# amin-abouee/apex-solver

Measured on AMD Instinct MI355X. Metric: ms per LM iter (Jacobian+Schur+solve), lower is better.
Workload: dtype f64; 1 GPU; final-13682 synthetic (13682 cameras / 4456117 landmarks / 28966251 observations); optimization_type=selfcal, camera_dof=9, schur_variant=sparse, s_tile_rows=856, s_tiles=8071, s_tiles_touched=4284, etree_levels=41, border_cameras=0, schur_form=4, variant_asked=Sparse, reason=, variant_choice=direct, parallelism=landmark-shard x1

## Files before the change

### apex-solver_amd/csrc/chol_kernels.hip

```cpp
#include <hip/hip_runtime.h>
#include <stdint.h>

#include "chol_kernels.h"
#include "device_reduce.hpp"
#include "tile_kernel_defs.h"
#include <algorithm>

namespace apex {

constexpr int BS = 16;
constexpr int NBK = NB / BS;
constexpr int BP = 18;
constexpr int BSZ = BS * BP;
constexpr int NLB = NBK * (NBK + 1) / 2;

__device__ __forceinline__ int bidx(int bi, int bj) { return bi * (bi + 1) / 2 + bj; }

__device__ __forceinline__ double readlane_f64(double v, int src) {
    const int lo = __builtin_amdgcn_readlane(__double2loint(v), src);
    const int hi = __builtin_amdgcn_readlane(__double2hiint(v), src);
    return __hiloint2double(hi, lo);
}

__device__ __forceinline__ double4_t blk_mma_nt(const double* X, const double* Y, double4_t acc, int lr, int lk, double sgn) {
// ... 176 lines not shown
                if (j + 2 < BS) {
                    const double dd = readlane_f64(Dm[(j + 2) >> 2], 16 * ((j + 2) & 3) + j + 2);
                    const double a0 = readlane_f64(l0, 16 * q0 + j + 2), a1 = readlane_f64(l1, 16 * q1 + j + 2);
                    dnext = fma(-a1, a1, fma(-a0, a0, dd));
                    Dm = __builtin_amdgcn_mfma_f64_16x16x4f64(-la, la, Dm, 0, 0, 0);
                    Xm = __builtin_amdgcn_mfma_f64_16x16x4f64(-la, xb, Xm, 0, 0, 0);
                }
            }
            double* D = sA + bidx(kb, kb) * BSZ;
            double* Xd = sD + kb * BSZ;
#pragma unroll
            for (int r = 0; r < 4; ++r) {
                const int c = lk + 4 * r;
                D[lr * BP + c] = lr >= c ? Ls[r] : 0.0;
                Xd[c * BP + lr] = Xs[r];
            }
            if (isbad) *bad = 1;
            POTRF_STAMP();
        } else if (helper) {
            if (kb >= 1) {
                const int ks = kb - 1;
                for (int i = kb + 1 + hid; i < NBK; i += NH) {
                    double* Cb = sA + bidx(i, kb) * BSZ;
                    double4_t acc = blk_load_cd(Cb, lr, lk);
                    acc = blk_mma_nt(sA + bidx(i, ks) * BSZ, sA + bidx(kb, ks) * BSZ, acc, lr, lk, -1.0);
                    blk_store_cd(Cb, acc, lr, lk, 1.0);
                }
                const int m = NBK - 1 - kb;
                const int n_upd = m * (m + 1) / 2;
                for (int t = hid; t < n_upd; t += NH) {
                    int ii = 0;
                    while ((ii + 1) * (ii + 2) / 2 <= t) ++ii;
                    const int jj = t - ii * (ii + 1) / 2;
                    const int i = kb + 1 + ii, j = kb + 1 + jj;
                    double* Cb = sA + bidx(i, j) * BSZ;
                    double4_t acc = blk_load_cd(Cb, lr, lk);
                    acc = blk_mma_nt(sA + bidx(i, ks) * BSZ, sA + bidx(j, ks) * BSZ, acc, lr, lk, -1.0);
                    blk_store_cd(Cb, acc, lr, lk, 1.0);
                }
                const int r = ks;
                int nt = 0;
                for (int j = hid; j < r; j += NH, ++nt) {
                    double4_t acc = (double4_t){0.0, 0.0, 0.0, 0.0};
                    for (int k = j; k < r; ++k) {
                        const double* Y = (k == j) ? (sD + j * BSZ) : (sA + bidx(k, j) * BSZ);
                        acc = blk_mma_nn(sA + bidx(r, k) * BSZ, Y, acc, lr, lk);
                    }
                    T[nt] = acc;
                }
            }
        }
        __syncthreads();
        POTRF_STAMP();
        if (helper && kb >= 1) {
            const int r = kb - 1;
            int nt = 0;
            for (int j = hid; j < r; j += NH, ++nt) blk_store_cd(sA + bidx(r, j) * BSZ, T[nt], lr, lk, -1.0);
        }
        {
            const int m = NBK - 1 - kb;
            if (w == 0) {
                if (m > 0) {
                    double* N = sA + bidx(kb + 1, kb) * BSZ;
                    double4_t Lt = (double4_t){0.0, 0.0, 0.0, 0.0};
                    Lt = blk_mma_nt(sD + kb * BSZ, N, Lt, lr, lk, 1.0);
                    Dm = blk_load_cd_sym(sA + bidx(kb + 1, kb + 1) * BSZ, lr, lk);
#pragma unroll
                    for (int r = 0; r < 4; ++r) N[lr * BP + lk + 4 * r] = Lt[r];
#pragma unroll
                    for (int r = 0; r < 4; ++r) Dm = __builtin_amdgcn_mfma_f64_16x16x4f64(-Lt[r], Lt[r], Dm, 0, 0, 0);
                }
            } else if (helper) {
                const int t0 = m > 0 ? 1 : 0;
                for (int t = t0 + hid; t < m + kb; t += NH) {
                    if (t < m) {
                        double* P = sA + bidx(kb + 1 + t, kb) * BSZ;
                        double4_t acc = (double4_t){0.0, 0.0, 0.0, 0.0};
                        acc = blk_mma_nt(P, sD + kb * BSZ, acc, lr, lk, 1.0);
                        blk_store_cd(P, acc, lr, lk, 1.0);
                    } else {
                        const int k = t - m;
                        double* Bk = sA + bidx(kb, k) * BSZ;
                        blk_to_tile<COH>(Bk, A, rA, kb, k, lane, 64);
                        double4_t acc = (double4_t){0.0, 0.0, 0.0, 0.0};
                        acc = blk_mma_nn(sD + kb * BSZ, Bk, acc, lr, lk);
                        blk_store_cd(Bk, acc, lr, lk, 1.0);
                    }
                }
                if (hid == NH - 1) blk_to_tile<COH>(sA + bidx(kb, kb) * BSZ, A, rA, kb, kb, lane, 64);
            }
        }
        if (w == 0 || helper) {
            __builtin_amdgcn_fence(__ATOMIC_RELEASE, "workgroup");
            if (lane == 0) __hip_atomic_fetch_add(sync_cnt, 1, __ATOMIC_RELAXED, __HIP_MEMORY_SCOPE_WORKGROUP);
        }
        if (helper) {
            const int target = (kb + 1) * (NH + 1);
            while (__hip_atomic_load(sync_cnt, __ATOMIC_RELAXED, __HIP_MEMORY_SCOPE_WORKGROUP) < target) __builtin_amdgcn_s_sleep(0);
            __builtin_amdgcn_fence(__ATOMIC_ACQUIRE, "workgroup");
        }
        POTRF_STAMP();
    }
    __syncthreads();
    {
        const int r = NBK - 1;
        double4_t T[(NBK - 1 + NW - 1) / NW];
        int nt = 0;
        for (int j = w; j < r; j += NW, ++nt) {
            double4_t acc = (double4_t){0.0, 0.0, 0.0, 0.0};
            for (int k = j; k < r; ++k) {
                const double* Y = (k == j) ? (sD + j * BSZ) : (sA + bidx(k, j) * BSZ);
                acc = blk_mma_nn(sA + bidx(r, k) * BSZ, Y, acc, lr, lk);
            }
            T[nt] = acc;
        }
        __syncthreads();
        nt = 0;
        for (int j = w; j < r; j += NW, ++nt) blk_store_cd(sA + bidx(r, j) * BSZ, T[nt], lr, lk, -1.0);
        __syncthreads();
    }
#pragma unroll
    for (int bi = 0; bi < NBK; ++bi) {
        const int per_row = 8 * (bi + 1), cnt = 16 * per_row;
        for (int idx = tid; idx < cnt; idx += NT) {
            const int rr = idx / per_row, c2 = idx - rr * per_row;
            const int bj = c2 >> 3;
            const double* src = ((bj == bi) ? (sD + bi * BSZ) : (sA + bidx(bi, bj) * BSZ)) + rr * BP + 2 * (c2 & 7);
            double2 v; v.x = src[0]; v.y = src[1];
            tile_st2<COH>(Linv, rL, (16 * bi + rr) * NB + 2 * c2, v);
        }
    }
    if (tid == 0 && *bad) atomicCAS(fail, 0, K + 1);
    POTRF_STAMP();
}

template <int NW>
__global__ __launch_bounds__(64 * NW) void k_potrf_inv_mf(const PotrfTask* __restrict__ tasks, int* __restrict__ fail,
                                                          int* __restrict__ arrived) {
    if (arrived != nullptr && threadIdx.x == 0) __hip_atomic_fetch_add(arrived, 1, __ATOMIC_RELAXED, __HIP_MEMORY_SCOPE_AGENT);
    POTRF_STAMP();
    __shared__ double sA[NLB * BSZ];
    __shared__ double sD[NBK * BSZ];
    __shared__ int bad, sync_cnt;
    const PotrfTask pt = tasks[blockIdx.x];
    potrf_tile_mf<NW, false>(pt.A, pt.Linv, pt.K, fail, sA, sD, &bad, &sync_cnt);
}
#undef POTRF_STAMP

constexpr int KC = 16;
constexpr int STRIP = 48;
constexpr int NSTRIP = NB / STRIP;
constexpr int kGemmSmallMax = 56;

template <bool TRI>
__global__ __launch_bounds__(256, 3) void k_tile_gemm_nt(const GemmTask* __restrict__ tasks, int n_units, double alpha, double beta) {
    constexpr int P4 = KC + 2;
    constexpr int IMG = (NB + STRIP) * P4;
    __shared__ double sm[IMG];
    const int per_xcd = (n_units + 7) >> 3;
    const int unit = (blockIdx.x & 7) * per_xcd + (blockIdx.x >> 3);
    if ((int)(blockIdx.x >> 3) >= per_xcd || unit >= n_units) return;
    GemmTask tg = tasks[unit / NSTRIP];
    const bool first = (reinterpret_cast<uintptr_t>(tg.C) & 1) != 0;
    tg.C = reinterpret_cast<double*>(reinterpret_cast<uintptr_t>(tg.C) & ~uintptr_t(7));
    const int strip = unit % NSTRIP;
    const int tid = threadIdx.x, lane = tid & 63, w = __builtin_amdgcn_readfirstlane(tid >> 6);
    const int lr = lane & 15, lk = lane >> 4;
    GlobalCF64 Ag = (GlobalCF64)tg.A + (size_t)strip * STRIP * NB;
    GlobalCF64 Bg = (GlobalCF64)tg.B;
    constexpr int NACC = TRI ? 9 : 7;
    int cb[3];
    if (TRI) { cb[0] = 16 * (8 - w); cb[1] = 16 * (1 + w); cb[2] = w == 3 ? 0 : -16; }
    else { cb[0] = 32 * w; cb[1] = 32 * w + 16; cb[2] = 128; }
    const bool extra = TRI ? (w == 3) : (w < 3);
    double4_t acc[NACC];
#pragma unroll
    for (int j = 0; j < NACC; ++j) acc[j] = (double4_t){0.0, 0.0, 0.0, 0.0};
    constexpr int C2 = KC / 2, NR = (NB + STRIP) * C2 / 256, RPR = 256 / C2;
    static_assert((NB + STRIP) * C2 % 256 == 0 && 256 % C2 == 0 && NR == 6 && RPR == 32, "staging loop assumes whole rounds");
    const int r0 = tid / C2, c2 = tid % C2;
    const unsigned offB = r0 * NB + 2 * c2, offA = (r0 + 16) * NB + 2 * c2;
    GlobalCF64 p4 = r0 < 16 ? Bg + (size_t)(r0 + 128) * NB + 2 * c2 : Ag + (size_t)(r0 - 16) * NB + 2 * c2;
    const int dst0 = r0 * P4 + 2 * c2;
    f64x2_t rg[NR];
    auto gload = [&](int k0) {
#pragma unroll
        for (int i = 0; i < 4; ++i) rg[i] = *reinterpret_cast<GlobalCF64x2>(Bg + (offB + (unsigned)(RPR * i * NB + k0)));
        rg[4] = *reinterpret_cast<GlobalCF64x2>(p4 + k0);
        rg[5] = *reinterpret_cast<GlobalCF64x2>(Ag + (offA + (unsigned)k0));
    };
    auto stage = [&](double* img) {
#pragma unroll
        for (int i = 0; i < NR; ++i) { img[dst0 + RPR * i * P4] = rg[i].x; img[dst0 + RPR * i * P4 + 1] = rg[i].y; }
    };
    auto compute = [&](const double* img, int k0) {
        const double* sB = img;
        const double* sA = img + NB * P4;
#pragma unroll
        for (int kk = 0; kk < KC; kk += 4) {
            if (TRI) {
                if (k0 > cb[0]) continue;
                double av[3], bv[3];
#pragma unroll
                for (int i = 0; i < 3; ++i) av[i] = sA[(16 * i + lr) * P4 + kk + lk];
#pragma unroll
                for (int j = 0; j < 3; ++j) bv[j] = sB[((cb[j] < 0 ? 0 : cb[j]) + lr) * P4 + kk + lk];
#pragma unroll
                for (int j = 0; j < 3; ++j) {
                    if (k0 > cb[j]) continue;
#pragma unroll
                    for (int i = 0; i < 3; ++i)
                        acc[3 * i + j] = __builtin_amdgcn_mfma_f64_16x16x4f64(av[i], bv[j], acc[3 * i + j], 0, 0, 0);
                }
            } else {
                double av[3], bv[2];
#pragma unroll
                for (int i = 0; i < 3; ++i) av[i] = sA[(16 * i + lr) * P4 + kk + lk];
#pragma unroll
                for (int j = 0; j < 2; ++j) bv[j] = sB[(cb[j] + lr) * P4 + kk + lk];
#pragma unroll
                for (int i = 0; i < 3; ++i)
#pragma unroll
                    for (int j = 0; j < 2; ++j)
                        acc[2 * i + j] = __builtin_amdgcn_mfma_f64_16x16x4f64(av[i], bv[j], acc[2 * i + j], 0, 0, 0);
                if (extra) {
                    const double ax = sA[(16 * w + lr) * P4 + kk + lk], bx = sB[(128 + lr) * P4 + kk + lk];
                    acc[6] = __builtin_amdgcn_mfma_f64_16x16x4f64(ax, bx, acc[6], 0, 0, 0);
                }
            }
        }
    };
    gload(0);
    for (int k0 = 0; k0 < NB; k0 += KC) {
        __syncthreads();
        stage(sm);
        __syncthreads();
        if (k0 + KC < NB) gload(k0 + KC);
        compute(sm, k0);
    }
    GlobalF64 C = (GlobalF64)tg.C + (size_t)strip * STRIP * NB;
    auto brow = [&](int n) { return TRI ? 16 * (n / 3) : (n < 6 ? 16 * (n / 2) : 16 * w); };
    auto bcol = [&](int n) { return TRI ? cb[n % 3] : (n < 6 ? cb[n % 2] : 128); };
    if (beta == 0.0 || first) {
        const double zero = first ? 0.0 : -0.0;
#pragma unroll
        for (int n = 0; n < NACC; ++n) {
            if (TRI ? (n % 3 == 2 && !extra) : (n == 6 && !extra)) continue;
#pragma unroll
            for (int r = 0; r < 4; ++r) C[(size_t)(brow(n) + lk + 4 * r) * NB + bcol(n) + lr] = alpha * acc[n][r] + zero;
        }
        return;
    }
    if (TRI) {
#pragma unroll
        for (int n = 0; n < NACC; ++n) {
            if (n % 3 == 2 && !extra) continue;
#pragma unroll
            for (int r = 0; r < 4; ++r) {
                GlobalF64 p = C + (size_t)(brow(n) + lk + 4 * r) * NB + bcol(n) + lr;
                *p = alpha * acc[n][r] + beta * *p;
            }
        }
        return;
    }
    double cv[3][4];
#pragma unroll
    for (int n = 0; n < 2; ++n)
#pragma unroll
        for (int r = 0; r < 4; ++r) cv[n][r] = C[(size_t)(brow(n) + lk + 4 * r) * NB + bcol(n) + lr];
#pragma unroll
    for (int n = 0; n < NACC; ++n) {
        if (n + 2 < NACC && (n + 2 < 6 || extra)) {
#pragma unroll
            for (int r = 0; r < 4; ++r) cv[(n + 2) % 3][r] = C[(size_t)(brow(n + 2) + lk + 4 * r) * NB + bcol(n + 2) + lr];
        }
        if (n == 6 && !extra) continue;
#pragma unroll
        for (int r = 0; r < 4; ++r)
            C[(size_t)(brow(n) + lk + 4 * r) * NB + bcol(n) + lr] = alpha * acc[n][r] + beta * cv[n % 3][r];
    }
}

__global__ __launch_bounds__(192) void k_tile_gemm_nt_small(const GemmTask* __restrict__ tasks, int n_units, double alpha,
                                                              double beta) {
    __shared__ double sA[48 * PS];
    __shared__ double sB[48 * PS];
    const int unit = blockIdx.x;
    if (unit >= n_units) return;
    GemmTask tg = tasks[unit / 9];
    const bool first = (reinterpret_cast<uintptr_t>(tg.C) & 1) != 0;
    tg.C = reinterpret_cast<double*>(reinterpret_cast<uintptr_t>(tg.C) & ~uintptr_t(7));
    if (first) beta = 0.0;
    const int blk = unit % 9, bi = blk / 3, bj = blk % 3;
    GlobalCF64 Ag = (GlobalCF64)tg.A + (size_t)bi * 48 * NB;
    GlobalCF64 Bg = (GlobalCF64)tg.B + (size_t)bj * 48 * NB;
    GlobalF64 C = (GlobalF64)tg.C + (size_t)bi * 48 * NB + bj * 48;
    const int tid = threadIdx.x, lane = tid & 63, w = tid >> 6;
    const int lr = lane & 15, lk = lane >> 4;
    double4_t acc[3];
#pragma unroll
    for (int j = 0; j < 3; ++j) acc[j] = (double4_t){0.0, 0.0, 0.0, 0.0};
    constexpr int C2 = KS / 2, NR = 48 * C2 / 192;
    static_assert(48 * C2 % 192 == 0 && NB % KS == 0, "staging loops assume whole rounds");
    f64x2_t ra[NR], rb[NR];
    auto gload = [&](int k0) {
#pragma unroll
        for (int i = 0; i < NR; ++i) {
            const int idx = tid + 192 * i, row = idx / C2, c2 = idx % C2;
            ra[i] = *reinterpret_cast<GlobalCF64x2>(Ag + (size_t)row * NB + k0 + 2 * c2);
            rb[i] = *reinterpret_cast<GlobalCF64x2>(Bg + (size_t)row * NB + k0 + 2 * c2);
        }
    };
    double cv[3][4];
    if (beta != 0.0) {
#pragma unroll
        for (int j = 0; j < 3; ++j)
#pragma unroll
            for (int r = 0; r < 4; ++r) cv[j][r] = C[(size_t)(16 * w + lk + 4 * r) * NB + 16 * j + lr];
    }
    gload(0);
    for (int k0 = 0; k0 < NB; k0 += KS) {
        __syncthreads();
#pragma unroll
        for (int i = 0; i < NR; ++i) {
            const int idx = tid + 192 * i, row = idx / C2, c2 = idx % C2;
            sA[row * PS + 2 * c2] = ra[i].x; sA[row * PS + 2 * c2 + 1] = ra[i].y;
            sB[row * PS + 2 * c2] = rb[i].x; sB[row * PS + 2 * c2 + 1] = rb[i].y;
        }
        __syncthreads();
        if (k0 + KS < NB) gload(k0 + KS);
#pragma unroll
        for (int kk = 0; kk < KS; kk += 4) {
            const double a = sA[(16 * w + lr) * PS + kk + lk];
#pragma unroll
            for (int j = 0; j < 3; ++j) {
                const double b = sB[(16 * j + lr) * PS + kk + lk];
                acc[j] = __builtin_amdgcn_mfma_f64_16x16x4f64(a, b, acc[j], 0, 0, 0);
            }
        }
    }
#pragma unroll
    for (int j = 0; j < 3; ++j)
#pragma unroll
        for (int r = 0; r < 4; ++r) {
            const double v = alpha * acc[j][r];
            C[(size_t)(16 * w + lk + 4 * r) * NB + 16 * j + lr] = (beta != 0.0) ? v + beta * cv[j][r] : (first ? v + 0.0 : v);
        }
}

__global__ __launch_bounds__(576) void k_tile_gemm_nt_small_strip(const GemmTask* __restrict__ tasks, int n_units, double alpha,
                                                                    double beta) {
    __shared__ double sA[48 * PS];
    __shared__ double sB[NB * PS];
    const int unit = blockIdx.x;
    if (unit >= n_units) return;
    const GemmTask tg = tasks[unit / 3];
    const int bi = unit % 3;
    GlobalCF64 Ag = (GlobalCF64)tg.A + (size_t)bi * 48 * NB;
    GlobalCF64 Bg = (GlobalCF64)tg.B;
    GlobalF64 C = (GlobalF64)tg.C + (size_t)bi * 48 * NB;
    const int tid = threadIdx.x, lane = tid & 63, w = tid >> 6;
    const int lr = lane & 15, lk = lane >> 4;
    const int wr = w / 3, wc = w % 3;
    double4_t acc[3];
#pragma unroll
    for (int j = 0; j < 3; ++j) acc[j] = (double4_t){0.0, 0.0, 0.0, 0.0};
    constexpr int C2 = KS / 2, NRA = 48 * C2 / 576, NRB = NB * C2 / 576;
    static_assert(48 * C2 % 576 == 0 && NB * C2 % 576 == 0, "staging loops assume whole rounds");
    f64x2_t ra[NRA], rb[NRB];
    auto gload = [&](int k0) {
#pragma unroll
        for (int i = 0; i < NRA; ++i) {
            const int idx = tid + 576 * i, row = idx / C2, c2 = idx % C2;
            ra[i] = *reinterpret_cast<GlobalCF64x2>(Ag + (size_t)row * NB + k0 + 2 * c2);
        }
#pragma unroll
        for (int i = 0; i < NRB; ++i) {
            const int idx = tid + 576 * i, row = idx / C2, c2 = idx % C2;
            rb[i] = *reinterpret_cast<GlobalCF64x2>(Bg + (size_t)row * NB + k0 + 2 * c2);
        }
// ... 308 lines not shown
            const double* __restrict__ pp = part + (size_t)t.part * NB + c;
            const double own = inl ? sinl[c] : 0.0;
            auto slot = [&](int q) { const double pv = flow_ld(pp + (size_t)q * NB); return q == s2 ? own : pv; };
            int q = g;
            for (; q + 12 < t.count; q += 16) {
                const double p0 = slot(q), p1 = slot(q + 4);
                const double p2 = slot(q + 8), p3 = slot(q + 12);
                v += (p0 + p1) + (p2 + p3);
            }
            for (; q < t.count; q += 4) v += slot(q);
        }
        spart[g][c] = v;
        __syncthreads();
        if (tid < NB) {
            const double* __restrict__ bsrc = t.src == -2 ? fold_b : b;
            const double rhs = bsrc ? bsrc[(size_t)t.dst * NB + tid] : 0.0;
            const double val = rhs - ((spart[0][tid] + spart[1][tid]) + (spart[2][tid] + spart[3][tid]));
            if (t.src == -2) fold_out[(size_t)t.dst * NB + tid] = val;
            else sx[tid] = val;
        }
        if (t.src == -2) return;
    }
    __syncthreads();
    double acc[kFwdRows];
    matvec(m, acc);
    if (cl == 15) {
        double* __restrict__ o = (t.src >= 0 ? part + (size_t)t.part * NB : y + (size_t)t.dst * NB) + row0;
#pragma unroll
        for (int rr = 0; rr < kFwdRows; ++rr) flow_st(o + rr, acc[rr]);
    }
    flow_publish(t.src >= 0 ? cnt + t.dst : done + t.dst, tid);
}

__device__ __forceinline__ void flow_wait_ge(const int* ver, int flag, int want, int tid, int* err) {
    if (flag >= 0) flow_wait(ver + flag, want, tid, err);
}
__device__ __forceinline__ void flow_wait_unit(const int* ver, const FactorUnit& u, int tid, int* err) {
    const int f0 = u.wait_flag[0], f1 = u.wait_flag[1], f2 = u.wait_flag[2], w0 = u.wait_val[0], w1 = u.wait_val[1], w2 = u.wait_val[2];
    if (tid < 64) {
        const int f = tid == 0 ? f0 : (tid == 1 ? f1 : (tid == 2 ? f2 : -1));
        const int want = tid == 0 ? w0 : (tid == 1 ? w1 : w2);
        int spins = 0;
        for (;;) {
            const bool ok = f < 0 || __hip_atomic_load(ver + f, __ATOMIC_RELAXED, __HIP_MEMORY_SCOPE_AGENT) >= want;
            if (__all(ok)) break;
            const bool dead = tid == 3 && __hip_atomic_load(err, __ATOMIC_RELAXED, __HIP_MEMORY_SCOPE_AGENT) != 0;
            if (__any(dead)) break;
            __builtin_amdgcn_s_sleep(1);
            if (++spins > kFlowSpinLimit) { if (tid == 0) atomicOr(err, 1); break; }
        }
    }
    __syncthreads();
}

constexpr int kFlowFactorThreadsC = 768;
constexpr int kFlowPK = NB + 2;
__device__ __forceinline__ void flow_update_unit(const FactorUnit& u, double* __restrict__ sA, double* __restrict__ sB,
                                                 int* __restrict__ ver, int* __restrict__ err, unsigned long long* __restrict__ trace) {
    const int tid = threadIdx.x, lane = tid & 63, w = tid >> 6;
    const int lr = lane & 15, lk = lane >> 4;
    const int wr = w / 3, wc = w % 3;
    const int bi = u.strip / 3, bj = u.strip % 3;
    const __amdgpu_buffer_rsrc_t rC = coh_rsrc(u.C), rA = coh_rsrc(u.A), rB = coh_rsrc(u.B);
    flow_wait_unit(ver, u, tid, err);
    if (trace && tid == 0) trace[1] = wall_clock64();
    const bool act = tid < 576;
    double cv[4] = {0.0, 0.0, 0.0, 0.0};
    if (act && !(u.kind & kFlowFirstWriter)) {
#pragma unroll
        for (int r = 0; r < 4; ++r) cv[r] = coh_ld1(rC, (48 * bi + 16 * wr + lk + 4 * r) * NB + 48 * bj + 16 * wc + lr);
    }
    constexpr int C2 = NB / 2, NR = 48 * C2 / 576;
    static_assert(48 * C2 % 576 == 0, "staging loops assume whole rounds");
    if (act) {
        double2 ra[NR], rb[NR];
#pragma unroll
        for (int i = 0; i < NR; ++i) {
            const int idx = tid + 576 * i, row = idx / C2, c2 = idx % C2;
            ra[i] = tile_ld2<true>(u.A, rA, (48 * bi + row) * NB + 2 * c2);
            rb[i] = tile_ld2<true>(u.B, rB, (48 * bj + row) * NB + 2 * c2);
        }
#pragma unroll
        for (int i = 0; i < NR; ++i) {
            const int idx = tid + 576 * i, row = idx / C2, c2 = idx % C2;
            sA[row * kFlowPK + 2 * c2] = ra[i].x; sA[row * kFlowPK + 2 * c2 + 1] = ra[i].y;
            sB[row * kFlowPK + 2 * c2] = rb[i].x; sB[row * kFlowPK + 2 * c2 + 1] = rb[i].y;
        }
    }
    __syncthreads();
    if (act) {
        double4_t acc = (double4_t){0.0, 0.0, 0.0, 0.0};
        const double* pa = sA + (16 * wr + lr) * kFlowPK + lk;
        const double* pb = sB + (16 * wc + lr) * kFlowPK + lk;
#pragma unroll
        for (int kk = 0; kk < NB; kk += 4) acc = __builtin_amdgcn_mfma_f64_16x16x4f64(pa[kk], pb[kk], acc, 0, 0, 0);
#pragma unroll
        for (int r = 0; r < 4; ++r)
            coh_st1(rC, (48 * bi + 16 * wr + lk + 4 * r) * NB + 48 * bj + 16 * wc + lr, -1.0 * acc[r] + 1.0 * cv[r]);
    }
    flow_publish(ver + u.pub, tid);
}

__device__ __forceinline__ void flow_solve_unit(const FactorUnit& u, double* __restrict__ sA, double* __restrict__ sB,
                                                int* __restrict__ ver, int* __restrict__ err, unsigned long long* __restrict__ trace) {
    const int tid = threadIdx.x, lane = tid & 63, w = tid >> 6;
    const int lr = lane & 15, lk = lane >> 4;
    const int row0 = 16 * u.strip;
    const __amdgpu_buffer_rsrc_t rC = coh_rsrc(u.C), rB = coh_rsrc(u.B);
    constexpr int C2 = KS / 2, NCH = NB / KS, NRB = NB * C2 / 576;
    static_assert(NB * C2 % 576 == 0 && 16 * C2 <= 576, "staging loops assume whole rounds");
    flow_wait_unit(ver, u, tid, err);
    if (trace && tid == 0) trace[1] = wall_clock64();
    const bool act = tid < 576;
    double2 ra[NCH], rb[NCH][NRB];
#pragma unroll
    for (int c = 0; c < NCH; ++c)
        if (tid < 16 * C2) ra[c] = tile_ld2<true>(u.C, rC, (row0 + tid / C2) * NB + KS * c + 2 * (tid % C2));
    if (act) {
#pragma unroll
        for (int c = 0; c < NCH; ++c)
#pragma unroll
            for (int i = 0; i < NRB; ++i) {
                const int idx = tid + 576 * i, row = idx / C2, c2 = idx % C2;
                rb[c][i] = tile_ld2<true>(u.B, rB, row * NB + KS * c + 2 * c2);
            }
    }
    double4_t acc = (double4_t){0.0, 0.0, 0.0, 0.0};
#pragma unroll
    for (int c = 0; c < NCH; ++c) {
        __syncthreads();
        if (tid < 16 * C2) { const int row = tid / C2, c2 = tid % C2; sA[row * PS + 2 * c2] = ra[c].x; sA[row * PS + 2 * c2 + 1] = ra[c].y; }
        if (act) {
#pragma unroll
            for (int i = 0; i < NRB; ++i) {
                const int idx = tid + 576 * i, row = idx / C2, c2 = idx % C2;
                sB[row * PS + 2 * c2] = rb[c][i].x; sB[row * PS + 2 * c2 + 1] = rb[c][i].y;
            }
        }
        __syncthreads();
        if (act) {
#pragma unroll
            for (int kk = 0; kk < KS; kk += 4)
                acc = __builtin_amdgcn_mfma_f64_16x16x4f64(sA[lr * PS + kk + lk], sB[(16 * w + lr) * PS + kk + lk], acc, 0, 0, 0);
        }
    }
    if (act) {
#pragma unroll
        for (int r = 0; r < 4; ++r) coh_st1(rC, (row0 + lk + 4 * r) * NB + 16 * w + lr, acc[r]);
    }
    flow_publish(ver + u.pub, tid);
}


__device__ __forceinline__ void flow_update_tile_unit(const FactorUnit& u, double* __restrict__ sA, double* __restrict__ sB,
                                                      int* __restrict__ ver, int* __restrict__ err, unsigned long long* __restrict__ trace) {
    const int tid = threadIdx.x, lane = tid & 63, w = tid >> 6;
    const int lr = lane & 15, lk = lane >> 4;
    const __amdgpu_buffer_rsrc_t rC = coh_rsrc(u.C), rA = coh_rsrc(u.A), rB = coh_rsrc(u.B);
    flow_wait_unit(ver, u, tid, err);
    if (trace && tid == 0) trace[1] = wall_clock64();
    constexpr int NBW = 7;
    const int nb = w < 9 ? 7 : 6, b0 = w < 9 ? 7 * w : 63 + 6 * (w - 9);
    constexpr int C2 = KS / 2, NCH = NB / KS;
    constexpr int NLD = (NB * C2 + kFlowFactorThreadsC - 1) / kFlowFactorThreadsC;
    double2 ra[NLD], rb[NLD];
    auto load_chunk = [&](int c) {
#pragma unroll
        for (int i = 0; i < NLD; ++i) {
            const int idx = tid + kFlowFactorThreadsC * i, row = min(idx / C2, NB - 1), c2 = idx % C2;
            ra[i] = tile_ld2<true>(u.A, rA, row * NB + KS * c + 2 * c2);
            rb[i] = tile_ld2<true>(u.B, rB, row * NB + KS * c + 2 * c2);
        }
    };
    load_chunk(0);
    double4_t acc[NBW];
#pragma unroll
    for (int q = 0; q < NBW; ++q) acc[q] = (double4_t){0.0, 0.0, 0.0, 0.0};
    double cv[NBW][4];
#pragma unroll
    for (int c = 0; c < NCH; ++c) {
        __syncthreads();
#pragma unroll
        for (int i = 0; i < NLD; ++i) {
            const int idx = tid + kFlowFactorThreadsC * i, row = idx / C2, c2 = idx % C2;
            if (idx < NB * C2) {
                sA[row * PS + 2 * c2] = ra[i].x; sA[row * PS + 2 * c2 + 1] = ra[i].y;
                sB[row * PS + 2 * c2] = rb[i].x; sB[row * PS + 2 * c2 + 1] = rb[i].y;
            }
        }
        if (c + 1 < NCH) {
            load_chunk(c + 1);
        } else {
            const bool first = (u.kind & kFlowFirstWriter) != 0;
#pragma unroll
            for (int q = 0; q < NBW; ++q) {
                const int b = min(b0 + q, 80), br = b / 9, bc = b - 9 * br;
#pragma unroll
                for (int r = 0; r < 4; ++r) cv[q][r] = first ? 0.0 : coh_ld1(rC, (16 * br + lk + 4 * r) * NB + 16 * bc + lr);
            }
        }
        __syncthreads();
#pragma unroll
        for (int q = 0; q < NBW; ++q) {
            if (q < nb) {
                const int b = b0 + q, br = b / 9, bc = b - 9 * br;
                const double* pa = sA + (16 * br + lr) * PS + lk;
                const double* pb = sB + (16 * bc + lr) * PS + lk;
#pragma unroll
                for (int kk = 0; kk < KS; kk += 4) acc[q] = __builtin_amdgcn_mfma_f64_16x16x4f64(pa[kk], pb[kk], acc[q], 0, 0, 0);
            }
        }
    }
#pragma unroll
    for (int q = 0; q < NBW; ++q) {
        if (q < nb) {
            const int b = b0 + q, br = b / 9, bc = b - 9 * br;
#pragma unroll
            for (int r = 0; r < 4; ++r) coh_st1(rC, (16 * br + lk + 4 * r) * NB + 16 * bc + lr, -1.0 * acc[q][r] + 1.0 * cv[q][r]);
        }
    }
    __builtin_amdgcn_s_waitcnt(0);
    __syncthreads();
    if (tid == 0) __hip_atomic_fetch_add(ver + u.pub, kFlowUnitsPerTile, __ATOMIC_RELAXED, __HIP_MEMORY_SCOPE_AGENT);
}

constexpr int kFlowFactorThreads = 768;
__global__ __launch_bounds__(kFlowFactorThreads) void k_factor_flow(const FactorUnit* __restrict__ units, int* __restrict__ ver,
                                                                     int* __restrict__ fail, int* __restrict__ err,
                                                                     unsigned long long* __restrict__ trace) {
    __shared__ double smem[(NLB + NBK) * BSZ];
    __shared__ int bad, sync_cnt;
    static_assert((16 + NB) * PS <= (NLB + NBK) * BSZ && 2 * 48 * kFlowPK <= (NLB + NBK) * BSZ && 2 * NB * PS <= (NLB + NBK) * BSZ, "the products' staging areas fit in the potrf's");
    static_assert(kFlowFactorThreadsC == kFlowFactorThreads, "one constant");
    const FactorUnit u = units[blockIdx.x];
    const int tid = threadIdx.x;
    if (trace) {
        trace += 3 * (size_t)blockIdx.x;
        if (tid == 0) trace[0] = wall_clock64();
    }
    const int kind = u.kind & 15;
    if (kind == 0) {
        flow_wait_unit(ver, u, tid, err);
        if (trace && tid == 0) trace[1] = wall_clock64();
        potrf_tile_mf<kFlowFactorThreads / 64, true>(u.C, const_cast<double*>(u.A), u.strip, fail, smem, smem + NLB * BSZ, &bad, &sync_cnt);
        __builtin_amdgcn_s_waitcnt(0);
        __syncthreads();
        if (tid == 0) __hip_atomic_fetch_add(ver + u.pub, kFlowUnitsPerTile, __ATOMIC_RELAXED, __HIP_MEMORY_SCOPE_AGENT);
    } else if (kind == 1) {
        flow_solve_unit(u, smem, smem + 16 * PS, ver, err, trace);
    } else if (kind == 3) {
        flow_update_tile_unit(u, smem, smem + NB * PS, ver, err, trace);
    } else {
        flow_update_unit(u, smem, smem + 48 * kFlowPK, ver, err, trace);
    }
    if (trace && tid == 0) trace[2] = wall_clock64();
}

__global__ __launch_bounds__(256) void k_tile_diag(const double* __restrict__ tiles, const int* __restrict__ diag_slot,
                                                     int nt, double* __restrict__ diag) {
    const int i = blockIdx.x * 256 + threadIdx.x;
    if (i >= nt * NB) return;
    const int I = i / NB, r = i - I * NB;
    diag[i] = tiles[(size_t)diag_slot[I] * (NB * NB) + (size_t)r * NB + r];
}

__global__ __launch_bounds__(256) void k_tile_add_diag(double* __restrict__ tiles, const int* __restrict__ diag_slot,
                                                         int n_valid, int n_total, double add_valid, double set_pad) {
    const int i = blockIdx.x * 256 + threadIdx.x;
    if (i >= n_total) return;
    const int I = i / NB, r = i - I * NB;
    double* d = tiles + (size_t)diag_slot[I] * (NB * NB) + (size_t)r * NB + r;
    if (i < n_valid) { if (add_valid != 0.0) *d += add_valid; }
    else *d = set_pad;
}

__global__ __launch_bounds__(256) void k_tile_scale_sym(const SymTile* __restrict__ list, double* __restrict__ tiles,
                                                          const double* __restrict__ scale) {
    const SymTile t = list[blockIdx.x];
    double* T = tiles + (size_t)t.slot * (NB * NB);
    const double* sr = scale + (size_t)t.I * NB;
    const double* sc = scale + (size_t)t.J * NB;
    for (int e = threadIdx.x; e < NB * NB; e += 256) {
        const int r = e / NB, c = e - r * NB;
        T[e] *= sr[r] * sc[c];
    }
}

__global__ __launch_bounds__(256) void k_vec_select(int n, const double* __restrict__ in, const int* __restrict__ cls, int mask,
                                                      double* __restrict__ out) {
    const int i = blockIdx.x * 256 + threadIdx.x;
    if (i < n) out[i] = ((mask >> cls[i / NB]) & 1) ? in[i] : 0.0;
}
__global__ __launch_bounds__(256) void k_vec_merge(int n, const double* __restrict__ src, const int* __restrict__ cls, int mask,
                                                     double* __restrict__ dst) {
    const int i = blockIdx.x * 256 + threadIdx.x;
    if (i < n && ((mask >> cls[i / NB]) & 1)) dst[i] = src[i];
}

__global__ __launch_bounds__(64) void k_gate(const int* __restrict__ arrived, int expected, long long max_ticks) {
    if (threadIdx.x != 0) return;
    const long long t0 = wall_clock64();
    while (__hip_atomic_load(arrived, __ATOMIC_RELAXED, __HIP_MEMORY_SCOPE_AGENT) < expected && wall_clock64() - t0 < max_ticks)
        __builtin_amdgcn_s_sleep(16);
}
void launch_gate(const int* arrived, int expected, int max_micros, hipStream_t s) {
    hipLaunchKernelGGL(k_gate, dim3(1), dim3(64), 0, s, arrived, expected, (long long)max_micros * 100);
}
void launch_factor_flow(const FactorUnit* units, int n_units, int* ver, int* fail, int* err, hipStream_t s, unsigned long long* trace) {
    if (n_units <= 0) return;
    hipLaunchKernelGGL(k_factor_flow, dim3(n_units), dim3(kFlowFactorThreads), 0, s, units, ver, fail, err, trace);
}
void launch_potrf_inv(const PotrfTask* tasks, int n, int* fail, hipStream_t s, int* arrived) {
    if (n <= 0) return;
    hipLaunchKernelGGL(k_potrf_inv_mf<12>, dim3(n), dim3(768), 0, s, tasks, fail, arrived);
}
void launch_tile_gemm_nt(const GemmTask* tasks, int n, double alpha, double beta, hipStream_t s, bool tri_b) {
    if (n <= 0) return;
    if (n <= kGemmSmallMax) {
        if (beta != 0.0) hipLaunchKernelGGL(k_tile_gemm_nt_small, dim3(9 * n), dim3(192), 0, s, tasks, 9 * n, alpha, beta);
        else hipLaunchKernelGGL(k_tile_gemm_nt_small_strip, dim3(3 * n), dim3(576), 0, s, tasks, 3 * n, alpha, beta);
        return;
    }
    const int units = n * NSTRIP, per_xcd = (units + 7) / 8;
    if (tri_b) hipLaunchKernelGGL(k_tile_gemm_nt<true>, dim3(8 * per_xcd), dim3(256), 0, s, tasks, units, alpha, beta);
    else hipLaunchKernelGGL(k_tile_gemm_nt<false>, dim3(8 * per_xcd), dim3(256), 0, s, tasks, units, alpha, beta);
}
void launch_tri_step(bool trans, const TriTask* tasks, int n, double* vwork, double* vout, hipStream_t s) {
    if (n <= 0) return;
    const int grid = 8 * ((n + 7) / 8);
    if (trans) hipLaunchKernelGGL(k_tri_step<true>, dim3(grid), dim3(256), 0, s, tasks, n, vwork, vout);
    else hipLaunchKernelGGL(k_tri_step<false>, dim3(grid), dim3(256), 0, s, tasks, n, vwork, vout);
}
__global__ __launch_bounds__(256) void k_occupy_cu(long long ticks_100mhz, int* started) {
    __shared__ char hog[156 * 1024];
    if (threadIdx.x == 0) {
        hog[blockIdx.x & 1023] = 1;
        __hip_atomic_fetch_add(started, 1, __ATOMIC_RELAXED, __HIP_MEMORY_SCOPE_SYSTEM);
        const long long t0 = (long long)__builtin_amdgcn_s_memrealtime();
        while ((long long)__builtin_amdgcn_s_memrealtime() - t0 < ticks_100mhz) __builtin_amdgcn_s_sleep(32);
        if (hog[(blockIdx.x + 7) & 1023] == 77) started[1] = 1;
    }
    __syncthreads();
}
void launch_occupy_cus(int n, int micros, int* started, hipStream_t s) {
    if (n > 0) hipLaunchKernelGGL(k_occupy_cu, dim3(n), dim3(256), 0, s, (long long)micros * 100, started);
}

__global__ __launch_bounds__(256) void k_clear_i32(int* __restrict__ p, int64_t n) {
    for (int64_t i = (int64_t)blockIdx.x * 256 + threadIdx.x; i < n; i += (int64_t)gridDim.x * 256) p[i] = 0;
}
void launch_clear_i32(int* p, int64_t n, hipStream_t s) {
    if (n <= 0) return;
    hipLaunchKernelGGL(k_clear_i32, dim3((unsigned)std::min<int64_t>(64, (n + 255) / 256)), dim3(256), 0, s, p, n);
}
__global__ void k_post_word(int* __restrict__ word, int* __restrict__ host_word) {
    const int v = word[0];
    if (v != 0) { host_word[0] = v; word[0] = 0; }
}
void launch_post_word(int* word, int* host_word_dev, hipStream_t s) { hipLaunchKernelGGL(k_post_word, dim3(1), dim3(1), 0, s, word, host_word_dev); }

void launch_tri_flow(bool backward, const FlowTask* tasks, int n_tasks, const double* in, double* out, double* part, int* flags,
                     int nt, hipStream_t s, const double* fold_b, double* fold_out, int poison_block, bool keep_flags) {
    if (n_tasks <= 0) return;
    if (!keep_flags) launch_clear_i32(flags, (int64_t)2 * nt, s);
    if (poison_block >= 0 && poison_block < nt)
        (void)hipMemsetD32Async(reinterpret_cast<hipDeviceptr_t>(flags + poison_block), (int)0x80000000, 1, s);
    int* err = flags + 2 * nt;
    if (backward) hipLaunchKernelGGL(k_tri_bwd_flow, dim3(n_tasks), dim3(kBwdThreads), 0, s, tasks, in, out, part, flags, flags + nt, err);
    else hipLaunchKernelGGL(k_tri_fwd_flow, dim3(n_tasks), dim3(kFwdThreads), 0, s, tasks, in, out, part, flags, flags + nt, err, fold_b, fold_out);
}
void launch_tile_diag(const double* tiles, const int* diag_slot, int nt, double* diag, hipStream_t s) {
    hipLaunchKernelGGL(k_tile_diag, dim3((nt * NB + 255) / 256), dim3(256), 0, s, tiles, diag_slot, nt, diag);
}
void launch_tile_add_diag(double* tiles, const int* diag_slot, int n_valid, int n_total, double add_valid,
                          double set_pad, hipStream_t s) {
    hipLaunchKernelGGL(k_tile_add_diag, dim3((n_total + 255) / 256), dim3(256), 0, s, tiles, diag_slot, n_valid, n_total, add_valid, set_pad);
}
void launch_vec_select(int n, const double* in, const int* cls, int mask, double* out, hipStream_t s) {
    if (n > 0) hipLaunchKernelGGL(k_vec_select, dim3((n + 255) / 256), dim3(256), 0, s, n, in, cls, mask, out);
}
void launch_vec_merge(int n, const double* src, const int* cls, int mask, double* dst, hipStream_t s) {
    if (n > 0) hipLaunchKernelGGL(k_vec_merge, dim3((n + 255) / 256), dim3(256), 0, s, n, src, cls, mask, dst);
}
void launch_tile_scale_sym(const SymTile* list, int n, double* tiles, const double* scale, hipStream_t s) {
    if (n > 0) hipLaunchKernelGGL(k_tile_scale_sym, dim3(n), dim3(256), 0, s, list, tiles, scale);
}

__global__ void k_warm_chol_kernels() {}
void warm_chol_kernels(hipStream_t s) { hipLaunchKernelGGL(k_warm_chol_kernels, dim3(1), dim3(64), 0, s); }

}
```

Baseline: 12.18 ms.

## Double-buffer flow tile update and reuse strip MFMA layout across waves

Rewrites the kind-3 tile update unit in the flow factor kernel. It now uses a double-buffered LDS image with a three-deep register prefetch of KC-wide chunks, and each group of four waves computes one 48-row strip using the same 3x2+extra MFMA block mapping as the non-triangular GEMM kernel (factored into a shared helper). This replaces the single-buffer, two-barrier scheme with 81 blocks spread unevenly over waves. It aims to overlap global loads with MFMA work and improve operand reuse, at the cost of more registers and LDS.

```diff
diff --git a/apex-solver_amd/csrc/chol_kernels.hip b/apex-solver_amd/csrc/chol_kernels.hip
--- a/apex-solver_amd/csrc/chol_kernels.hip
+++ b/apex-solver_amd/csrc/chol_kernels.hip
@@ -352,9 +352,34 @@
 constexpr int NSTRIP = NB / STRIP;
 constexpr int kGemmSmallMax = 56;
 
+constexpr int kStripPitch = KC + 2;
+__device__ __forceinline__ void strip_chunk_mma(const double* __restrict__ sA, const double* __restrict__ sB, int w, int lr, int lk,
+                                                double4_t* __restrict__ acc) {
+    constexpr int P4 = kStripPitch;
+    const int cb0 = 32 * w, cb1 = 32 * w + 16;
+    const bool extra = w < 3;
+#pragma unroll
+    for (int kk = 0; kk < KC; kk += 4) {
+        double av[3], bv[2];
+#pragma unroll
+        for (int i = 0; i < 3; ++i) av[i] = sA[(16 * i + lr) * P4 + kk + lk];
+        bv[0] = sB[(cb0 + lr) * P4 + kk + lk];
+        bv[1] = sB[(cb1 + lr) * P4 + kk + lk];
+#pragma unroll
+        for (int i = 0; i < 3; ++i)
+#pragma unroll
+            for (int j = 0; j < 2; ++j)
+                acc[2 * i + j] = __builtin_amdgcn_mfma_f64_16x16x4f64(av[i], bv[j], acc[2 * i + j], 0, 0, 0);
+        if (extra) {
+            const double ax = sA[(16 * w + lr) * P4 + kk + lk], bx = sB[(128 + lr) * P4 + kk + lk];
+            acc[6] = __builtin_amdgcn_mfma_f64_16x16x4f64(ax, bx, acc[6], 0, 0, 0);
+        }
+    }
+}
+
 template <bool TRI>
 __global__ __launch_bounds__(256, 3) void k_tile_gemm_nt(const GemmTask* __restrict__ tasks, int n_units, double alpha, double beta) {
-    constexpr int P4 = KC + 2;
+    constexpr int P4 = kStripPitch;
     constexpr int IMG = (NB + STRIP) * P4;
     __shared__ double sm[IMG];
     const int per_xcd = (n_units + 7) >> 3;
@@ -396,9 +421,11 @@
     auto compute = [&](const double* img, int k0) {
         const double* sB = img;
         const double* sA = img + NB * P4;
-#pragma unroll
-        for (int kk = 0; kk < KC; kk += 4) {
-            if (TRI) {
+        if constexpr (!TRI) {
+            strip_chunk_mma(sA, sB, w, lr, lk, acc);
+        } else {
+#pragma unroll
+            for (int kk = 0; kk < KC; kk += 4) {
                 if (k0 > cb[0]) continue;
                 double av[3], bv[3];
 #pragma unroll
@@ -411,21 +438,6 @@
 #pragma unroll
                     for (int i = 0; i < 3; ++i)
                         acc[3 * i + j] = __builtin_amdgcn_mfma_f64_16x16x4f64(av[i], bv[j], acc[3 * i + j], 0, 0, 0);
-                }
-            } else {
-                double av[3], bv[2];
-#pragma unroll
-                for (int i = 0; i < 3; ++i) av[i] = sA[(16 * i + lr) * P4 + kk + lk];
-#pragma unroll
-                for (int j = 0; j < 2; ++j) bv[j] = sB[(cb[j] + lr) * P4 + kk + lk];
-#pragma unroll
-                for (int i = 0; i < 3; ++i)
-#pragma unroll
-                    for (int j = 0; j < 2; ++j)
-                        acc[2 * i + j] = __builtin_amdgcn_mfma_f64_16x16x4f64(av[i], bv[j], acc[2 * i + j], 0, 0, 0);
-                if (extra) {
-                    const double ax = sA[(16 * w + lr) * P4 + kk + lk], bx = sB[(128 + lr) * P4 + kk + lk];
-                    acc[6] = __builtin_amdgcn_mfma_f64_16x16x4f64(ax, bx, acc[6], 0, 0, 0);
                 }
             }
         }
@@ -1040,72 +1052,68 @@
 }
 
 
-__device__ __forceinline__ void flow_update_tile_unit(const FactorUnit& u, double* __restrict__ sA, double* __restrict__ sB,
+__device__ __forceinline__ void flow_update_tile_unit(const FactorUnit& u, double* __restrict__ sm,
                                                       int* __restrict__ ver, int* __restrict__ err, unsigned long long* __restrict__ trace) {
-    const int tid = threadIdx.x, lane = tid & 63, w = tid >> 6;
+    const int tid = threadIdx.x, lane = tid & 63, w = __builtin_amdgcn_readfirstlane(tid >> 6);
     const int lr = lane & 15, lk = lane >> 4;
+    const int strip = w >> 2, q = (w + strip) & 3;
     const __amdgpu_buffer_rsrc_t rC = coh_rsrc(u.C), rA = coh_rsrc(u.A), rB = coh_rsrc(u.B);
     flow_wait_unit(ver, u, tid, err);
     if (trace && tid == 0) trace[1] = wall_clock64();
+    constexpr int P4 = kStripPitch, IMG = 2 * NB * P4, NCH = NB / KC;
+    constexpr int C2 = KC / 2, NR = 2 * NB * C2 / kFlowFactorThreadsC, RPR = kFlowFactorThreadsC / C2;
+    static_assert(2 * NB * C2 % kFlowFactorThreadsC == 0 && kFlowFactorThreadsC % C2 == 0 && NR == 3 && RPR == 96, "staging loop assumes whole rounds");
+    const int r0 = tid / C2, c2 = tid % C2;
+    const bool lowB = w < 6;
+    const __amdgpu_buffer_rsrc_t r1 = lowB ? rB : rA;
+    const double* t1 = lowB ? u.B : u.A;
+    const int off0 = r0 * NB + 2 * c2, off1 = (lowB ? r0 + 96 : r0 - 48) * NB + 2 * c2, off2 = (r0 + 48) * NB + 2 * c2;
+    const int dst0 = r0 * P4 + 2 * c2;
+    double2 rg[2][NR];
+    auto gload = [&](int n) {
+        rg[n & 1][0] = tile_ld2<true>(u.B, rB, off0 + KC * n);
+        rg[n & 1][1] = tile_ld2<true>(t1, r1, off1 + KC * n);
+        rg[n & 1][2] = tile_ld2<true>(u.A, rA, off2 + KC * n);
+    };
+    auto stage = [&](int n) {
+        double* img = sm + (n & 1) * IMG;
+#pragma unroll
+        for (int i = 0; i < NR; ++i) { img[dst0 + RPR * i * P4] = rg[n & 1][i].x; img[dst0 + RPR * i * P4 + 1] = rg[n & 1][i].y; }
+    };
+    auto brow = [&](int n) { return STRIP * strip + (n < 6 ? 16 * (n / 2) : 16 * q); };
+    auto bcol = [&](int n) { return n < 6 ? 32 * q + 16 * (n % 2) : 128; };
     constexpr int NBW = 7;
-    const int nb = w < 9 ? 7 : 6, b0 = w < 9 ? 7 * w : 63 + 6 * (w - 9);
-    constexpr int C2 = KS / 2, NCH = NB / KS;
-    constexpr int NLD = (NB * C2 + kFlowFactorThreadsC - 1) / kFlowFactorThreadsC;
-    double2 ra[NLD], rb[NLD];
-    auto load_chunk = [&](int c) {
-#pragma unroll
-        for (int i = 0; i < NLD; ++i) {
-            const int idx = tid + kFlowFactorThreadsC * i, row = min(idx / C2, NB - 1), c2 = idx % C2;
-            ra[i] = tile_ld2<true>(u.A, rA, row * NB + KS * c + 2 * c2);
-            rb[i] = tile_ld2<true>(u.B, rB, row * NB + KS * c + 2 * c2);
-        }
-    };
-    load_chunk(0);
+    const bool extra = q < 3;
     double4_t acc[NBW];
 #pragma unroll
-    for (int q = 0; q < NBW; ++q) acc[q] = (double4_t){0.0, 0.0, 0.0, 0.0};
+    for (int n = 0; n < NBW; ++n) acc[n] = (double4_t){0.0, 0.0, 0.0, 0.0};
     double cv[NBW][4];
+    gload(0);
+    gload(1);
+    stage(0);
+    gload(2);
 #pragma unroll
     for (int c = 0; c < NCH; ++c) {
         __syncthreads();
-#pragma unroll
-        for (int i = 0; i < NLD; ++i) {
-            const int idx = tid + kFlowFactorThreadsC * i, row = idx / C2, c2 = idx % C2;
-            if (idx < NB * C2) {
-                sA[row * PS + 2 * c2] = ra[i].x; sA[row * PS + 2 * c2 + 1] = ra[i].y;
-                sB[row * PS + 2 * c2] = rb[i].x; sB[row * PS + 2 * c2 + 1] = rb[i].y;
-            }
-        }
-        if (c + 1 < NCH) {
-            load_chunk(c + 1);
-        } else {
+        const double* img = sm + (c & 1) * IMG;
+        strip_chunk_mma(img + (NB + STRIP * strip) * P4, img, q, lr, lk, acc);
+        if (c + 1 < NCH) stage(c + 1);
+        if (c + 3 < NCH) {
+            gload(c + 3);
+        } else if (c + 3 == NCH) {
             const bool first = (u.kind & kFlowFirstWriter) != 0;
 #pragma unroll
-            for (int q = 0; q < NBW; ++q) {
-                const int b = min(b0 + q, 80), br = b / 9, bc = b - 9 * br;
-#pragma unroll
-                for (int r = 0; r < 4; ++r) cv[q][r] = first ? 0.0 : coh_ld1(rC, (16 * br + lk + 4 * r) * NB + 16 * bc + lr);
-            }
-        }
-        __syncthreads();
-#pragma unroll
-        for (int q = 0; q < NBW; ++q) {
-            if (q < nb) {
-                const int b = b0 + q, br = b / 9, bc = b - 9 * br;
-                const double* pa = sA + (16 * br + lr) * PS + lk;
-                const double* pb = sB + (16 * bc + lr) * PS + lk;
-#pragma unroll
-                for (int kk = 0; kk < KS; kk += 4) acc[q] = __builtin_amdgcn_mfma_f64_16x16x4f64(pa[kk], pb[kk], acc[q], 0, 0, 0);
-            }
-        }
-    }
-#pragma unroll
-    for (int q = 0; q < NBW; ++q) {
-        if (q < nb) {
-            const int b = b0 + q, br = b / 9, bc = b - 9 * br;
-#pragma unroll
-            for (int r = 0; r < 4; ++r) coh_st1(rC, (16 * br + lk + 4 * r) * NB + 16 * bc + lr, -1.0 * acc[q][r] + 1.0 * cv[q][r]);
-        }
+            for (int n = 0; n < NBW; ++n)
+#pragma unroll
+                for (int r = 0; r < 4; ++r)
+                    cv[n][r] = (first || (n == 6 && !extra)) ? 0.0 : coh_ld1(rC, (brow(n) + lk + 4 * r) * NB + bcol(n) + lr);
+        }
+    }
+#pragma unroll
+    for (int n = 0; n < NBW; ++n) {
+        if (n == 6 && !extra) continue;
+#pragma unroll
+        for (int r = 0; r < 4; ++r) coh_st1(rC, (brow(n) + lk + 4 * r) * NB + bcol(n) + lr, -1.0 * acc[n][r] + 1.0 * cv[n][r]);
     }
     __builtin_amdgcn_s_waitcnt(0);
     __syncthreads();
@@ -1118,7 +1126,7 @@
                                                                      unsigned long long* __restrict__ trace) {
     __shared__ double smem[(NLB + NBK) * BSZ];
     __shared__ int bad, sync_cnt;
-    static_assert((16 + NB) * PS <= (NLB + NBK) * BSZ && 2 * 48 * kFlowPK <= (NLB + NBK) * BSZ && 2 * NB * PS <= (NLB + NBK) * BSZ, "the products' staging areas fit in the potrf's");
+    static_assert((16 + NB) * PS <= (NLB + NBK) * BSZ && 2 * 48 * kFlowPK <= (NLB + NBK) * BSZ && 4 * NB * kStripPitch <= (NLB + NBK) * BSZ, "the products' staging areas fit in the potrf's");
     static_assert(kFlowFactorThreadsC == kFlowFactorThreads, "one constant");
     const FactorUnit u = units[blockIdx.x];
     const int tid = threadIdx.x;
@@ -1137,7 +1145,7 @@
     } else if (kind == 1) {
         flow_solve_unit(u, smem, smem + 16 * PS, ver, err, trace);
     } else if (kind == 3) {
-        flow_update_tile_unit(u, smem, smem + NB * PS, ver, err, trace);
+        flow_update_tile_unit(u, smem, ver, err, trace);
     } else {
         flow_update_unit(u, smem, smem + 48 * kFlowPK, ver, err, trace);
     }
```

New measurement: 12.19 ms, median of 2. No clear change (+0.0%).
